# Qervas/cn_chess_ai

Measured on AMD Instinct MI355X. Metric: env steps/sec + DQN updates/sec at 8192 parallel games, 1/2/4/8 MI355X, higher is better.
Workload: dtype f32

## Files before the change

### cn_chess_ai_amd/csrc/xq_refine.hip.h

```cpp
#pragma once

namespace xq {

constexpr float kScreenEps = 0.0078125f * 1.0625f;
constexpr float kScreenBiasEps = 0.001953125f;
enum { kScreenCheckEvery = 32, kScreenHoldSteps = 512 };
constexpr double kScreenMaxPairs = 24.0, kScreenMaxWhole = 1.0;

__device__ __forceinline__ int float_order_key(float f) {
    const int b = __builtin_bit_cast(int, f);
    return b ^ ((b >> 31) & 0x7fffffff);
}
__device__ __forceinline__ float float_from_key(int k) { return __builtin_bit_cast(float, k ^ ((k >> 31) & 0x7fffffff)); }
__device__ __forceinline__ float wave_sum_f32(float v) {
#pragma unroll
    for (int off = 32; off >= 1; off >>= 1) v += __shfl_xor(v, off, 64);
    return v;
}

enum { kRefineSamples = 32, kRefineMaxPerThread = 64 };

template <int KFIX>
__device__ __forceinline__ float quarter_dot(const float* __restrict__ ap, const float* __restrict__ wp, int K, int ql) {
    float acc = 0.f;
    if (KFIX > 0) {
        constexpr int NT = KFIX > 0 ? KFIX / 64 : 1;
        float4 x[NT], w[NT];
#pragma unroll
        for (int t = 0; t < KFIX / 64; ++t) {
            x[t] = *reinterpret_cast<const float4*>(ap + t * 64 + ql * 4);
            w[t] = *reinterpret_cast<const float4*>(wp + t * 64 + ql * 4);
        }
#pragma unroll
        for (int t = 0; t < KFIX / 64; ++t) {
            acc = fmaf(x[t].x, w[t].x, acc); acc = fmaf(x[t].y, w[t].y, acc);
            acc = fmaf(x[t].z, w[t].z, acc); acc = fmaf(x[t].w, w[t].w, acc);
        }
    } else {
        for (int k = ql * 4; k < K; k += 64) {
            const float4 x = *reinterpret_cast<const float4*>(ap + k);
            const float4 w = *reinterpret_cast<const float4*>(wp + k);
            acc = fmaf(x.x, w.x, acc); acc = fmaf(x.y, w.y, acc); acc = fmaf(x.z, w.z, acc); acc = fmaf(x.w, w.w, acc);
        }
    }
    return acc;
}
__device__ __forceinline__ float quarter_sum(float v) {
#pragma unroll
    for (int off = 8; off >= 1; off >>= 1) v += __shfl_xor(v, off, 64);
    return v;
}
__device__ __forceinline__ int screen_row(int g, int code) {
    const int q = code & 15;
    return (g >> 2) * 128 + ((g >> 1) & 1) * 64 + 4 * (g & 1) + (code >> 4) * 32 + (q & 3) + 8 * (q >> 2);
}

template <int KFIX, int NPT>
__global__ __launch_bounds__(256) void qmax_refine_kernel(const float* __restrict__ P1, const float* __restrict__ P2, int G, int n, long long ldp,
                                                          const float* __restrict__ a_last, int K, const float* __restrict__ W,
                                                          const float* __restrict__ bias, int NO, unsigned* __restrict__ wm, int parity,
                                                          float* __restrict__ zmax, unsigned long long* __restrict__ stats) {
    extern __shared__ __attribute__((aligned(16))) uint32_t cand[];
    uint16_t* wlist = reinterpret_cast<uint16_t*>(cand + (size_t)G * kRefineSamples);
    __shared__ float sv[8][32];
    __shared__ float na[32], thr[32];
    __shared__ int best[32];
    __shared__ int cnt, nexp;
    const int tid = (int)threadIdx.x;
    const int sl = tid & 31, phase = tid >> 5;
    const int ql = tid & 15, quarter = tid >> 4;
    const int b0 = (int)blockIdx.x * kRefineSamples;
    const int b = b0 + sl;
    const bool ok = b < n;
    if (tid == 0) { cnt = 0; nexp = 0; if (blockIdx.x == 0) { wm[parity ^ 1] = 0u; wm[2 + (parity ^ 1)] = 0u; } }
    unsigned long long st_pairs = 0, st_whole = 0;
    if (tid == 0) { st_pairs = stats[2 * blockIdx.x]; st_whole = stats[2 * blockIdx.x + 1]; }
    if (tid < 32) best[tid] = (int)0x80000000;
    float v[NPT], v2[NPT];
    const int bc = min(b, n - 1);
#pragma unroll
    for (int u = 0; u < NPT; ++u) {
        const int g = min(phase + 8 * u, G - 1);
        v[u] = P1[(long long)g * ldp + bc];
        v2[u] = P2[(long long)g * ldp + bc];
    }
#pragma unroll
    for (int u = 0; u < NPT; ++u)
        if (!ok || phase + 8 * u >= G) { v[u] = kColmaxPadBias; v2[u] = kColmaxPadBias; }
#pragma unroll
    for (int r = 0; r < 2; ++r) {
        const int i = quarter + 16 * r;
        const float* ap = a_last + (long long)min(b0 + i, n - 1) * K;
        const float ss = quarter_sum(quarter_dot<KFIX>(ap, ap, K, ql));
        if (ql == 0) na[i] = ss;
    }
    float m = kColmaxPadBias;
#pragma unroll
    for (int u = 0; u < NPT; ++u) m = fmaxf(m, v[u]);
    sv[phase][sl] = m;
    __syncthreads();
    if (tid < 32) {
        m = sv[0][sl];
#pragma unroll
        for (int p = 1; p < 8; ++p) m = fmaxf(m, sv[p][sl]);
        const float wmx = fmaxf(__builtin_bit_cast(float, wm[parity]), __builtin_bit_cast(float, wm[4]));
        const float bmx = fmaxf(__builtin_bit_cast(float, wm[2 + parity]), __builtin_bit_cast(float, wm[5]));
        const float B = kScreenEps * sqrtf(na[sl]) * wmx + kScreenBiasEps * bmx;
        float t0 = m - 2.f * B * 1.03125f - 1.52587890625e-05f * (fabsf(m) + 2.f * B);
        if (!(t0 == t0)) t0 = -__builtin_inff();
        thr[sl] = b0 + sl < n ? t0 : __builtin_inff();
    }
    __syncthreads();
    {
        const float t = thr[sl];
#pragma unroll
        for (int u = 0; u < NPT; ++u) {
            const int g = phase + 8 * u;
            if (v[u] >= t) {
                if (v2[u] >= t) wlist[atomicAdd(&nexp, 1)] = (uint16_t)(sl | (g << 5));
                else cand[atomicAdd(&cnt, 1)] = (uint32_t)sl | ((uint32_t)screen_row(g, (int)(__builtin_bit_cast(uint32_t, v[u]) & 31u)) << 5);
            }
        }
    }
    __syncthreads();
    const int singles = cnt, wholes = nexp;
    for (int e0 = 0; e0 < singles; e0 += 64) {
        float z[4];
        int s2[4], row[4];
        bool live[4];
#pragma unroll
        for (int r = 0; r < 4; ++r) {
            const int e = e0 + quarter + 16 * r;
            live[r] = e < singles;
            const uint32_t ent = cand[live[r] ? e : 0];
            s2[r] = (int)(ent & 31u);
            row[r] = min((int)(ent >> 5), NO - 1);
            z[r] = quarter_dot<KFIX>(a_last + (long long)(b0 + s2[r]) * K, W + (long long)row[r] * K, K, ql);
        }
#pragma unroll
        for (int r = 0; r < 4; ++r) {
            z[r] = quarter_sum(z[r]) + bias[row[r]];
            if (live[r] && ql == 0 && z[r] == z[r]) atomicMax(&best[s2[r]], float_order_key(z[r]));
        }
    }
    for (int e = 0; e < wholes; ++e) {
        const int ent = wlist[e];
        const int s2 = ent & 31, g = ent >> 5;
        float zb = kColmaxPadBias;
#pragma unroll
        for (int r = 0; r < 2; ++r) {
            const int row = screen_row(g, quarter + 16 * r);
            const int rc = min(row, NO - 1);
            const float z = quarter_sum(quarter_dot<KFIX>(a_last + (long long)(b0 + s2) * K, W + (long long)rc * K, K, ql)) + bias[rc];
            if (row < NO) zb = fmaxf(zb, z);
        }
        if (ql == 0) atomicMax(&best[s2], float_order_key(zb));
    }
    __syncthreads();
    if (tid < 32 && ok) zmax[b] = float_from_key(best[sl]);
    if (tid == 0) {
        stats[2 * blockIdx.x] = st_pairs + (unsigned long long)(singles + wholes);
        stats[2 * blockIdx.x + 1] = st_whole + (unsigned long long)wholes;
    }
}

struct TdFused {
    SlotSrc src;
    const int32_t* action_to; const float* reward; const uint8_t* done;
    const float* a_s;
    const float* w_out; const float* b_out;
    const float* view; long long view_ld; int view_kmax;
    float gamma;
    float* dtop; float* dsc; int32_t* act; float* qsa; float* yv; float* lossv;
};
__host__ __device__ inline size_t refine_cand_words(int G) { const size_t w = (size_t)G * 32; return w < 8192 ? 8192 : w; }
__host__ __device__ inline size_t refine_wlist_bytes(int G) { return ((size_t)G * 32 * sizeof(uint16_t) + 15) & ~(size_t)15; }
__host__ __device__ inline size_t refine_stage_bytes() { return (size_t)3 * 32 * 256 * sizeof(float); }
template <int KFIX, bool TD = false, class Loss = SquaredLoss>
__global__ __launch_bounds__(256) void qmax_refine2_kernel(const float* __restrict__ R, int ranges, int gpr ,
                                                           const float* __restrict__ P1, const float* __restrict__ P2, int G, int n, long long ldp,
                                                           const float* __restrict__ na_all, const float* __restrict__ a_last, int K,
                                                           const float* __restrict__ W, const float* __restrict__ bias, int NO,
                                                           unsigned* __restrict__ wm, int parity, float* __restrict__ zmax,
                                                           unsigned long long* __restrict__ stats, const TdFused T, int whole_mode, const Loss L) {
    extern __shared__ __attribute__((aligned(16))) uint32_t cand[];
    uint16_t* wlist = reinterpret_cast<uint16_t*>(cand + refine_cand_words(G));
    __shared__ float sv[8][32];
    __shared__ float thr[32];
    __shared__ int best[32];
    __shared__ int cnt, nexp;
    __shared__ unsigned gbits[256];
    __shared__ unsigned long long gpop[4];
    const int tid = (int)threadIdx.x;
    const int sl = tid & 31, phase = tid >> 5;
    const int ql = tid & 15, quarter = tid >> 4;
    const int b0 = (int)blockIdx.x * kRefineSamples;
    const int b = b0 + sl;
    const bool ok = b < n;
    const int bc = min(b, n - 1);
    if (tid == 0) { cnt = 0; nexp = 0; if (blockIdx.x == 0) { wm[parity ^ 1] = 0u; wm[2 + (parity ^ 1)] = 0u; } }
    unsigned long long st_pairs = 0, st_whole = 0;
    if (tid == 0) { st_pairs = stats[2 * blockIdx.x]; st_whole = stats[2 * blockIdx.x + 1]; }
    if (tid < 32) best[tid] = (int)0x80000000;
    const bool stage_ok = KFIX > 0 && G <= 256;
    gbits[tid] = 0u;
    const int td_lane = tid & 63, td_w = tid >> 6;
    int td_a = -1; float td_r = 0.f, td_bo = 0.f; bool td_dn = false;
    float zq[8];
    if (TD) {
        static_assert(!TD || KFIX == 256, "fused TD delta: 256-wide last hidden layer");
        if (td_lane < 8) {
            const int bb = min(b0 + td_w * 8 + td_lane, n - 1);
            const int sslot = slot_of(T.src, bb);
            td_a = T.action_to[sslot];
            td_r = T.reward[sslot];
            td_dn = T.done[sslot] != 0;
            td_bo = T.b_out[(td_a >= 0 && td_a < 96) ? td_a : 0];
        }
#pragma unroll
        for (int i = 0; i < 8; ++i) {
            const int bb = min(b0 + td_w * 8 + i, n - 1);
            const int a = __shfl(td_a, i, 64);
            const int ac = (a >= 0 && a < 96) ? a : 0;
            const float4 av = *reinterpret_cast<const float4*>(T.a_s + (long long)bb * 256 + td_lane * 4);
            const float4 wv = *reinterpret_cast<const float4*>(T.w_out + (long long)ac * 256 + td_lane * 4);
            zq[i] = (av.x * wv.x + av.y * wv.y) + (av.z * wv.z + av.w * wv.w);
        }
    }
    float m = kColmaxPadBias;
    for (int r = phase; r < ranges; r += 8) m = fmaxf(m, R[(long long)r * ldp + bc]);
    sv[phase][sl] = m;
    __syncthreads();
    if (tid < 32) {
        m = sv[0][sl];
#pragma unroll
        for (int p = 1; p < 8; ++p) m = fmaxf(m, sv[p][sl]);
        const float wmx = fmaxf(__builtin_bit_cast(float, wm[parity]), __builtin_bit_cast(float, wm[4]));
        const float bmx = fmaxf(__builtin_bit_cast(float, wm[2 + parity]), __builtin_bit_cast(float, wm[5]));
        const float B = kScreenEps * sqrtf(na_all[bc]) * wmx + kScreenBiasEps * bmx;
        float t0 = m - 2.f * B * 1.03125f - 1.52587890625e-05f * (fabsf(m) + 2.f * B);
        if (!(t0 == t0)) t0 = -__builtin_inff();
        thr[sl] = ok ? t0 : __builtin_inff();
    }
    __syncthreads();
    {
        const float t = thr[sl];
        for (int r = phase; r < ranges; r += 8) {
            if (R[(long long)r * ldp + bc] < t) continue;
            const int g0 = r * gpr, g1 = min(G, g0 + gpr);
            for (int g = g0; g < g1; g += 16) {
                float v[16], v2[16];
#pragma unroll
                for (int u = 0; u < 16; ++u) v[u] = P1[(long long)min(g + u, g1 - 1) * ldp + bc];
#pragma unroll
                for (int u = 0; u < 16; ++u) v2[u] = (g + u < g1 && v[u] >= t) ? P2[(long long)(g + u) * ldp + bc] : 0.f;
#pragma unroll
                for (int u = 0; u < 16; ++u) {
                    if (g + u < g1 && v[u] >= t) {
                        if (v2[u] >= t) { wlist[atomicAdd(&nexp, 1)] = (uint16_t)(sl | ((g + u) << 5)); if (stage_ok) atomicOr(&gbits[g + u], 1u << sl); }
                        else cand[atomicAdd(&cnt, 1)] = (uint32_t)sl | ((uint32_t)screen_row(g + u, (int)(__builtin_bit_cast(uint32_t, v[u]) & 31u)) << 5);
                    }
                }
            }
        }
    }
    __syncthreads();
    const int singles = cnt, wholes = nexp;
    for (int e0 = 0; e0 < singles; e0 += 64) {
        float z[4];
        int s2[4], row[4];
        bool live[4];
#pragma unroll
        for (int r = 0; r < 4; ++r) {
            const int e = e0 + quarter + 16 * r;
            live[r] = e < singles;
            const uint32_t ent = cand[live[r] ? e : 0];
            s2[r] = (int)(ent & 31u);
            row[r] = min((int)(ent >> 5), NO - 1);
            z[r] = quarter_dot<KFIX>(a_last + (long long)(b0 + s2[r]) * K, W + (long long)row[r] * K, K, ql);
        }
#pragma unroll
        for (int r = 0; r < 4; ++r) {
            z[r] = quarter_sum(z[r]) + bias[row[r]];
            if (live[r] && ql == 0 && z[r] == z[r]) atomicMax(&best[s2[r]], float_order_key(z[r]));
        }
    }
    const bool staged_pass = stage_ok && KFIX == 256 && wholes >= 8 && whole_mode == 2;
    if (staged_pass) {
        float* Wt0 = reinterpret_cast<float*>(cand);
        float* At = reinterpret_cast<float*>(reinterpret_cast<unsigned char*>(wlist) + refine_wlist_bytes(G));
        {
            const unsigned long long m = __ballot(__popc(gbits[tid]) >= 8);
            if ((tid & 63) == 0) gpop[tid >> 6] = m;
        }
        __syncthreads();
        unsigned long long gm[4] = {gpop[0], gpop[1], gpop[2], gpop[3]};
        bool a_staged = false;
        for (;;) {
            int gs[3];
#pragma unroll
            for (int u = 0; u < 3; ++u) {
                gs[u] = -1;
#pragma unroll
                for (int wv = 0; wv < 4; ++wv)
                    if (gs[u] < 0 && gm[wv]) { gs[u] = wv * 64 + __builtin_ctzll(gm[wv]); gm[wv] &= gm[wv] - 1; }
            }
            if (gs[0] < 0) break;
            float bj[3][2];
#pragma unroll
            for (int u = 0; u < 3; ++u)
#pragma unroll
                for (int r = 0; r < 2; ++r) bj[u][r] = gs[u] >= 0 ? bias[min(screen_row(gs[u], quarter + 16 * r), NO - 1)] : 0.f;
#pragma unroll
            for (int half = 0; half < 2; ++half) {
                float4 ra[4], rw0[4], rw1[4], rw2[4];
#pragma unroll
                for (int q = 0; q < 4; ++q) {
                    const int i = (half * 4 + q) * 256 + tid, j = i >> 6, c = i & 63;
                    ra[q] = *reinterpret_cast<const float4*>(a_last + (long long)min(b0 + j, n - 1) * K + 4 * c);
                    rw0[q] = *reinterpret_cast<const float4*>(W + (long long)min(screen_row(gs[0], j), NO - 1) * K + 4 * c);
                    rw1[q] = *reinterpret_cast<const float4*>(W + (long long)min(screen_row(gs[1] >= 0 ? gs[1] : gs[0], j), NO - 1) * K + 4 * c);
                    rw2[q] = *reinterpret_cast<const float4*>(W + (long long)min(screen_row(gs[2] >= 0 ? gs[2] : gs[0], j), NO - 1) * K + 4 * c);
                }
#pragma unroll
                for (int q = 0; q < 4; ++q) {
                    const int i = (half * 4 + q) * 256 + tid;
                    if (!a_staged) reinterpret_cast<float4*>(At)[i] = ra[q];
                    if (gs[0] >= 0) reinterpret_cast<float4*>(Wt0)[i] = rw0[q];
                    if (gs[1] >= 0) reinterpret_cast<float4*>(At + 1 * 32 * 256)[i] = rw1[q];
                    if (gs[2] >= 0) reinterpret_cast<float4*>(At + 2 * 32 * 256)[i] = rw2[q];
                }
            }
            a_staged = true;
            __syncthreads();
#pragma unroll
            for (int u = 0; u < 3; ++u) {
                if (gs[u] < 0) continue;
                const float* Wt = u == 0 ? Wt0 : At + u * 32 * 256;
                unsigned left = gbits[gs[u]];
                while (left) {
                    const int s2 = __builtin_ctz(left);
                    left &= left - 1;
                    float zb = kColmaxPadBias;
#pragma unroll
                    for (int r = 0; r < 2; ++r) {
                        const int j = quarter + 16 * r;
                        const float z = quarter_sum(quarter_dot<KFIX>(At + s2 * 256, Wt + j * 256, K, ql)) + bj[u][r];
                        if (screen_row(gs[u], j) < NO) zb = fmaxf(zb, z);
                    }
                    if (ql == 0) atomicMax(&best[s2], float_order_key(zb));
                }
            }
            __syncthreads();
        }
    }
    for (int e = 0; e < wholes; ++e) {
        const int ent = wlist[e];
        const int s2 = ent & 31, g = ent >> 5;
        if (staged_pass && __popc(gbits[g]) >= 8) continue;
        float zb = kColmaxPadBias;
#pragma unroll
        for (int r = 0; r < 2; ++r) {
            const int row = screen_row(g, quarter + 16 * r);
            const int rc = min(row, NO - 1);
            const float z = quarter_sum(quarter_dot<KFIX>(a_last + (long long)(b0 + s2) * K, W + (long long)rc * K, K, ql)) + bias[rc];
            if (row < NO) zb = fmaxf(zb, z);
        }
        if (ql == 0) atomicMax(&best[s2], float_order_key(zb));
    }
    __syncthreads();
    if (tid < 32 && ok) zmax[b] = float_from_key(best[sl]);
    if (tid == 0) {
        stats[2 * blockIdx.x] = st_pairs + (unsigned long long)(singles + wholes);
        stats[2 * blockIdx.x + 1] = st_whole + (unsigned long long)wholes;
    }
    if (TD) {
        float4 av[8], vv[8];
#pragma unroll
        for (int i = 0; i < 8; ++i) {
            const int bb = min(b0 + td_w * 8 + i, n - 1);
            const int a = __shfl(td_a, i, 64);
            const bool has_view = a >= 0 && a < 96 && a < T.view_kmax;
            av[i] = *reinterpret_cast<const float4*>(T.a_s + (long long)bb * 256 + td_lane * 4);
            vv[i] = has_view ? *reinterpret_cast<const float4*>(T.view + (long long)a * T.view_ld + td_lane * 4) : make_float4(0.f, 0.f, 0.f, 0.f);
        }
#pragma unroll
        for (int i = 0; i < 8; ++i) {
            const int bb = b0 + td_w * 8 + i;
            const int a = __shfl(td_a, i, 64);
            const float r = __shfl(td_r, i, 64), bo = __shfl(td_bo, i, 64);
            const bool dn = __shfl((int)td_dn, i, 64) != 0;
            const bool live = a >= 0 && a < 96;
            float z = zq[i];
#pragma unroll
            for (int off = 32; off > 0; off >>= 1) z += __shfl_xor(z, off, 64);
            const float zm = float_from_key(best[td_w * 8 + i]);
            float q = 0.f, y = 0.f, delta = 0.f;
            if (live) {
                q = tanhf(z + bo);
                y = dn ? r : r + T.gamma * tanhf(zm);
                delta = L.err(q - y) * td_dtanh(q) * 1.f;
            }
            if (bb < n) {
                float4 o = make_float4(0.f, 0.f, 0.f, 0.f);
                if (live && a < T.view_kmax) {
                    o.x = delta * vv[i].x * (1.f - av[i].x * av[i].x); o.y = delta * vv[i].y * (1.f - av[i].y * av[i].y);
                    o.z = delta * vv[i].z * (1.f - av[i].z * av[i].z); o.w = delta * vv[i].w * (1.f - av[i].w * av[i].w);
                }
                *reinterpret_cast<float4*>(T.dtop + (long long)bb * 256 + td_lane * 4) = o;
                if (td_lane == 0) {
                    T.dsc[bb] = delta;
                    T.act[bb] = live ? a : -1;
                    T.qsa[bb] = q; T.yv[bb] = y;
                    T.lossv[bb] = live ? L.loss(q - y) : 0.f;
                }
            }
        }
    }
}


}
```

Measured before the change: 47.85 million.

## Restructure refine kernel to hoist loads, drop a barrier, and batch screening reads

Result: faster. 48.75 million, median of 6 (+1.9%).

```diff
diff --git a/cn_chess_ai_amd/csrc/xq_refine.hip.h b/cn_chess_ai_amd/csrc/xq_refine.hip.h
--- a/cn_chess_ai_amd/csrc/xq_refine.hip.h
+++ b/cn_chess_ai_amd/csrc/xq_refine.hip.h
@@ -176,7 +176,43 @@
 __host__ __device__ inline size_t refine_cand_words(int G) { const size_t w = (size_t)G * 32; return w < 8192 ? 8192 : w; }
 __host__ __device__ inline size_t refine_wlist_bytes(int G) { return ((size_t)G * 32 * sizeof(uint16_t) + 15) & ~(size_t)15; }
 __host__ __device__ inline size_t refine_stage_bytes() { return (size_t)3 * 32 * 256 * sizeof(float); }
-template <int KFIX, bool TD = false, class Loss = SquaredLoss>
+#ifdef XQ_REFINE_PROBE
+__device__ unsigned long long* refine_dbg;
+__device__ __forceinline__ unsigned long long refine_clock() {
+    unsigned long long t;
+    asm volatile("s_waitcnt vmcnt(0) lgkmcnt(0)\n\ts_memtime %0\n\ts_waitcnt lgkmcnt(0)" : "=s"(t) :: "memory");
+    return t;
+}
+__device__ __forceinline__ unsigned long long refine_realtime() { return __builtin_amdgcn_s_memrealtime(); }
+__device__ __forceinline__ void refine_stamp_out(int k, unsigned long long v) { refine_dbg[(size_t)blockIdx.x * 16 + k] = v; }
+#else
+__device__ __forceinline__ unsigned long long refine_clock() { return 0ull; }
+__device__ __forceinline__ unsigned long long refine_realtime() { return 0ull; }
+__device__ __forceinline__ void refine_stamp_out(int, unsigned long long) {}
+#endif
+struct RefineChunk { float v[16], w[16]; };
+__device__ __forceinline__ unsigned refine_chunk_last(bool on, int g, int g1) { return on && g1 > g ? (unsigned)(g1 - 1 - g) : 0u; }
+__device__ __forceinline__ void refine_chunk_p1(RefineChunk& c, const float* __restrict__ P1s, bool on, int g, int g1, unsigned ld) {
+    const float* base = P1s + (unsigned long long)(unsigned)(on && g1 > g ? g : 0) * ld;
+    const unsigned last = refine_chunk_last(on, g, g1);
+#pragma unroll
+    for (unsigned u = 0; u < 16; ++u) c.v[u] = base[(unsigned long long)min(u, last) * ld];
+}
+template <bool EAGER>
+__device__ __forceinline__ void refine_chunk_p2(RefineChunk& c, const float* __restrict__ P2s, bool on, int g, int g1, unsigned ld, float t) {
+    const float* base = P2s + (unsigned long long)(unsigned)(on && g1 > g ? g : 0) * ld;
+    const unsigned last = refine_chunk_last(on, g, g1);
+#pragma unroll
+    for (unsigned u = 0; u < 16; ++u) {
+        if (EAGER) c.w[u] = base[(unsigned long long)min(u, last) * ld];
+        else c.w[u] = base[(unsigned long long)((u <= last && c.v[u] >= t) ? u : 0u) * ld];
+    }
+}
+__device__ __forceinline__ void refine_chunk_pin(float (&x)[16]) {
+#pragma unroll
+    for (int u = 0; u < 16; ++u) asm volatile("" : "+v"(x[u]));
+}
+template <int KFIX, bool TD = false, class Loss = SquaredLoss, int DBG = 0>
 __global__ __launch_bounds__(256) void qmax_refine2_kernel(const float* __restrict__ R, int ranges, int gpr ,
                                                            const float* __restrict__ P1, const float* __restrict__ P2, int G, int n, long long ldp,
                                                            const float* __restrict__ na_all, const float* __restrict__ a_last, int K,
@@ -186,18 +222,28 @@
     extern __shared__ __attribute__((aligned(16))) uint32_t cand[];
     uint16_t* wlist = reinterpret_cast<uint16_t*>(cand + refine_cand_words(G));
     __shared__ float sv[8][32];
-    __shared__ float thr[32];
     __shared__ int best[32];
     __shared__ int cnt, nexp;
     __shared__ unsigned gbits[256];
     __shared__ unsigned long long gpop[4];
     const int tid = (int)threadIdx.x;
+    unsigned long long stp[13] = {0, 0, 0, 0, 0, 0, 0, 0, 0, 0, 0, 0, 0};
+    if (DBG & 1) { stp[11] = refine_realtime(); stp[0] = refine_clock(); }
     const int sl = tid & 31, phase = tid >> 5;
     const int ql = tid & 15, quarter = tid >> 4;
     const int b0 = (int)blockIdx.x * kRefineSamples;
     const int b = b0 + sl;
     const bool ok = b < n;
     const int bc = min(b, n - 1);
+    const bool two = ranges <= 16 && gpr <= 16;
+    float r0 = kColmaxPadBias, r1 = kColmaxPadBias;
+    float m = kColmaxPadBias;
+    if (two) {
+        r0 = R[(long long)min(phase, ranges - 1) * ldp + bc];
+        r1 = R[(long long)min(phase + 8, ranges - 1) * ldp + bc];
+    }
+    const float na_b = na_all[bc];
+    const unsigned wm_w = wm[parity], wm_ws = wm[4], wm_b = wm[2 + parity], wm_bs = wm[5];
     if (tid == 0) { cnt = 0; nexp = 0; if (blockIdx.x == 0) { wm[parity ^ 1] = 0u; wm[2 + (parity ^ 1)] = 0u; } }
     unsigned long long st_pairs = 0, st_whole = 0;
     if (tid == 0) { st_pairs = stats[2 * blockIdx.x]; st_whole = stats[2 * blockIdx.x + 1]; }
@@ -205,8 +251,7 @@
     const bool stage_ok = KFIX > 0 && G <= 256;
     gbits[tid] = 0u;
     const int td_lane = tid & 63, td_w = tid >> 6;
-    int td_a = -1; float td_r = 0.f, td_bo = 0.f; bool td_dn = false;
-    float zq[8];
+    int td_a = -1; float td_r = 0.f, td_bo = 0.f; unsigned td_dn = 0u;
     if (TD) {
         static_assert(!TD || KFIX == 256, "fused TD delta: 256-wide last hidden layer");
         if (td_lane < 8) {
@@ -214,60 +259,118 @@
             const int sslot = slot_of(T.src, bb);
             td_a = T.action_to[sslot];
             td_r = T.reward[sslot];
-            td_dn = T.done[sslot] != 0;
-            td_bo = T.b_out[(td_a >= 0 && td_a < 96) ? td_a : 0];
-        }
+            td_dn = T.done[sslot];
+        }
+    }
+    if (two) {
+        if (phase < ranges) m = fmaxf(m, r0);
+        if (phase + 8 < ranges) m = fmaxf(m, r1);
+    } else {
+        for (int r = phase; r < ranges; r += 8) m = fmaxf(m, R[(long long)r * ldp + bc]);
+    }
+    sv[phase][sl] = m;
+    if (DBG & 1) stp[1] = refine_clock();
+    __syncthreads();
+    if (DBG & 1) stp[2] = refine_clock();
+    float4 tav[8], twv[8], tvv[8];
+    if (TD) {
+        if (td_lane < 8) td_bo = T.b_out[(td_a >= 0 && td_a < 96) ? td_a : 0];
 #pragma unroll
         for (int i = 0; i < 8; ++i) {
             const int bb = min(b0 + td_w * 8 + i, n - 1);
             const int a = __shfl(td_a, i, 64);
             const int ac = (a >= 0 && a < 96) ? a : 0;
-            const float4 av = *reinterpret_cast<const float4*>(T.a_s + (long long)bb * 256 + td_lane * 4);
-            const float4 wv = *reinterpret_cast<const float4*>(T.w_out + (long long)ac * 256 + td_lane * 4);
-            zq[i] = (av.x * wv.x + av.y * wv.y) + (av.z * wv.z + av.w * wv.w);
-        }
-    }
-    float m = kColmaxPadBias;
-    for (int r = phase; r < ranges; r += 8) m = fmaxf(m, R[(long long)r * ldp + bc]);
-    sv[phase][sl] = m;
-    __syncthreads();
-    if (tid < 32) {
+            const float* vp = (a >= 0 && a < 96 && a < T.view_kmax) ? T.view + (long long)a * T.view_ld : T.w_out;
+            tav[i] = *reinterpret_cast<const float4*>(T.a_s + (long long)bb * 256 + td_lane * 4);
+            twv[i] = *reinterpret_cast<const float4*>(T.w_out + (long long)ac * 256 + td_lane * 4);
+            tvv[i] = *reinterpret_cast<const float4*>(vp + td_lane * 4);
+        }
+    }
+    if (DBG & 1) stp[3] = refine_clock();
+    float t;
+    {
         m = sv[0][sl];
 #pragma unroll
         for (int p = 1; p < 8; ++p) m = fmaxf(m, sv[p][sl]);
-        const float wmx = fmaxf(__builtin_bit_cast(float, wm[parity]), __builtin_bit_cast(float, wm[4]));
-        const float bmx = fmaxf(__builtin_bit_cast(float, wm[2 + parity]), __builtin_bit_cast(float, wm[5]));
-        const float B = kScreenEps * sqrtf(na_all[bc]) * wmx + kScreenBiasEps * bmx;
+        const float wmx = fmaxf(__builtin_bit_cast(float, wm_w), __builtin_bit_cast(float, wm_ws));
+        const float bmx = fmaxf(__builtin_bit_cast(float, wm_b), __builtin_bit_cast(float, wm_bs));
+        const float B = kScreenEps * sqrtf(na_b) * wmx + kScreenBiasEps * bmx;
         float t0 = m - 2.f * B * 1.03125f - 1.52587890625e-05f * (fabsf(m) + 2.f * B);
         if (!(t0 == t0)) t0 = -__builtin_inff();
-        thr[sl] = ok ? t0 : __builtin_inff();
-    }
-    __syncthreads();
+        t = ok ? t0 : __builtin_inff();
+    }
     {
-        const float t = thr[sl];
-        for (int r = phase; r < ranges; r += 8) {
-            if (R[(long long)r * ldp + bc] < t) continue;
-            const int g0 = r * gpr, g1 = min(G, g0 + gpr);
-            for (int g = g0; g < g1; g += 16) {
-                float v[16], v2[16];
-#pragma unroll
-                for (int u = 0; u < 16; ++u) v[u] = P1[(long long)min(g + u, g1 - 1) * ldp + bc];
-#pragma unroll
-                for (int u = 0; u < 16; ++u) v2[u] = (g + u < g1 && v[u] >= t) ? P2[(long long)(g + u) * ldp + bc] : 0.f;
-#pragma unroll
-                for (int u = 0; u < 16; ++u) {
-                    if (g + u < g1 && v[u] >= t) {
-                        if (v2[u] >= t) { wlist[atomicAdd(&nexp, 1)] = (uint16_t)(sl | ((g + u) << 5)); if (stage_ok) atomicOr(&gbits[g + u], 1u << sl); }
-                        else cand[atomicAdd(&cnt, 1)] = (uint32_t)sl | ((uint32_t)screen_row(g + u, (int)(__builtin_bit_cast(uint32_t, v[u]) & 31u)) << 5);
-                    }
-                }
-            }
-        }
-    }
-    __syncthreads();
+        const float *P1s = P1 + bc, *P2s = P2 + bc;
+        const unsigned ld = (unsigned)ldp;
+        const auto emit = [&](const RefineChunk& c, bool on, int g, int g1) {
+#pragma unroll
+            for (int u = 0; u < 16; ++u) {
+                if (on && g + u < g1 && c.v[u] >= t) {
+                    if (c.w[u] >= t) { wlist[atomicAdd(&nexp, 1)] = (uint16_t)(sl | ((g + u) << 5)); if (stage_ok) atomicOr(&gbits[g + u], 1u << sl); }
+                    else cand[atomicAdd(&cnt, 1)] = (uint32_t)sl | ((uint32_t)screen_row(g + u, (int)(__builtin_bit_cast(uint32_t, c.v[u]) & 31u)) << 5);
+                }
+            }
+        };
+        constexpr bool EAGER = (DBG & 2) != 0;
+        if (two) {
+            const bool hit0 = phase < ranges && !(r0 < t), hit1 = phase + 8 < ranges && !(r1 < t);
+            const int ga = phase * gpr, gb = (phase + 8) * gpr;
+            const int ea = hit0 ? min(G, ga + gpr) : ga, eb = hit1 ? min(G, gb + gpr) : gb;
+            if (hit0 || hit1) {
+                RefineChunk ca, cb;
+                refine_chunk_p1(ca, P1s, hit0, ga, ea, ld);
+                refine_chunk_p1(cb, P1s, hit1, gb, eb, ld);
+                if (EAGER) { refine_chunk_p2<true>(ca, P2s, hit0, ga, ea, ld, t); refine_chunk_p2<true>(cb, P2s, hit1, gb, eb, ld, t); }
+                __builtin_amdgcn_sched_barrier(0);
+                if (DBG & 1) stp[4] = refine_clock();
+                refine_chunk_pin(ca.v); refine_chunk_pin(cb.v);
+                if (!EAGER) {
+                    refine_chunk_p2<false>(ca, P2s, hit0, ga, ea, ld, t); refine_chunk_p2<false>(cb, P2s, hit1, gb, eb, ld, t);
+                    __builtin_amdgcn_sched_barrier(0);
+                }
+                if (DBG & 1) stp[5] = refine_clock();
+                refine_chunk_pin(ca.w); refine_chunk_pin(cb.w);
+                emit(ca, hit0, ga, ea);
+                emit(cb, hit1, gb, eb);
+            }
+        } else {
+            for (int r = phase; r < ranges; r += 8) {
+                if (R[(long long)r * ldp + bc] < t) continue;
+                const int g0 = r * gpr, g1 = min(G, g0 + gpr);
+                for (int g = g0; g < g1; g += 16) {
+                    RefineChunk c;
+                    refine_chunk_p1(c, P1s, true, g, g1, ld);
+                    refine_chunk_pin(c.v);
+                    refine_chunk_p2<EAGER>(c, P2s, true, g, g1, ld, t);
+                    refine_chunk_pin(c.w);
+                    emit(c, true, g, g1);
+                }
+            }
+#if defined(__HIP_DEVICE_COMPILE__) && !defined(__gfx950__)
+#error "qmax_refine2_kernel: the s_waitcnt immediate below is encoded for gfx950"
+#endif
+            __builtin_amdgcn_s_waitcnt(0x0F70);
+        }
+    }
+    if (DBG & 1) { stp[6] = refine_clock(); if (stp[4] == 0) stp[4] = stp[5] = stp[6]; }
+    float td_q = 0.f;
+    if (TD) {
+        float zmine = 0.f;
+#pragma unroll
+        for (int i = 0; i < 8; ++i) {
+            const float4 av = tav[i], wv = twv[i];
+            float z = (av.x * wv.x + av.y * wv.y) + (av.z * wv.z + av.w * wv.w);
+#pragma unroll
+            for (int off = 32; off > 0; off >>= 1) z += __shfl_xor(z, off, 64);
+            if (td_lane == i) zmine = z;
+        }
+        if (td_lane < 8 && td_a >= 0 && td_a < 96) td_q = tanhf(zmine + td_bo);
+    }
+    __syncthreads();
+    if (DBG & 1) stp[7] = refine_clock();
     const int singles = cnt, wholes = nexp;
     for (int e0 = 0; e0 < singles; e0 += 64) {
-        float z[4];
+        float z[4], bj[4];
         int s2[4], row[4];
         bool live[4];
 #pragma unroll
@@ -277,14 +380,16 @@
             const uint32_t ent = cand[live[r] ? e : 0];
             s2[r] = (int)(ent & 31u);
             row[r] = min((int)(ent >> 5), NO - 1);
+            bj[r] = bias[row[r]];
             z[r] = quarter_dot<KFIX>(a_last + (long long)(b0 + s2[r]) * K, W + (long long)row[r] * K, K, ql);
         }
 #pragma unroll
         for (int r = 0; r < 4; ++r) {
-            z[r] = quarter_sum(z[r]) + bias[row[r]];
+            z[r] = quarter_sum(z[r]) + bj[r];
             if (live[r] && ql == 0 && z[r] == z[r]) atomicMax(&best[s2[r]], float_order_key(z[r]));
         }
     }
+    if (DBG & 1) stp[8] = refine_clock();
     const bool staged_pass = stage_ok && KFIX == 256 && wholes >= 8 && whole_mode == 2;
     if (staged_pass) {
         float* Wt0 = reinterpret_cast<float*>(cand);
@@ -359,65 +464,67 @@
         const int s2 = ent & 31, g = ent >> 5;
         if (staged_pass && __popc(gbits[g]) >= 8) continue;
         float zb = kColmaxPadBias;
+        float bj[2];
+#pragma unroll
+        for (int r = 0; r < 2; ++r) bj[r] = bias[min(screen_row(g, quarter + 16 * r), NO - 1)];
 #pragma unroll
         for (int r = 0; r < 2; ++r) {
             const int row = screen_row(g, quarter + 16 * r);
             const int rc = min(row, NO - 1);
-            const float z = quarter_sum(quarter_dot<KFIX>(a_last + (long long)(b0 + s2) * K, W + (long long)rc * K, K, ql)) + bias[rc];
+            const float z = quarter_sum(quarter_dot<KFIX>(a_last + (long long)(b0 + s2) * K, W + (long long)rc * K, K, ql)) + bj[r];
             if (row < NO) zb = fmaxf(zb, z);
         }
         if (ql == 0) atomicMax(&best[s2], float_order_key(zb));
     }
     __syncthreads();
+    if (DBG & 1) stp[9] = refine_clock();
     if (tid < 32 && ok) zmax[b] = float_from_key(best[sl]);
     if (tid == 0) {
         stats[2 * blockIdx.x] = st_pairs + (unsigned long long)(singles + wholes);
         stats[2 * blockIdx.x + 1] = st_whole + (unsigned long long)wholes;
     }
     if (TD) {
-        float4 av[8], vv[8];
-#pragma unroll
-        for (int i = 0; i < 8; ++i) {
-            const int bb = min(b0 + td_w * 8 + i, n - 1);
-            const int a = __shfl(td_a, i, 64);
-            const bool has_view = a >= 0 && a < 96 && a < T.view_kmax;
-            av[i] = *reinterpret_cast<const float4*>(T.a_s + (long long)bb * 256 + td_lane * 4);
-            vv[i] = has_view ? *reinterpret_cast<const float4*>(T.view + (long long)a * T.view_ld + td_lane * 4) : make_float4(0.f, 0.f, 0.f, 0.f);
+        const bool mine = td_a >= 0 && td_a < 96;
+        float q = 0.f, y = 0.f, delta = 0.f;
+        if (td_lane < 8) {
+            const float zm = float_from_key(best[td_w * 8 + td_lane]);
+            const float r = td_r;
+            const bool dn = td_dn != 0u;
+            if (mine) {
+                q = td_q;
+                y = dn ? r : r + T.gamma * tanhf(zm);
+                delta = L.err(q - y) * td_dtanh(q) * 1.f;
+            }
+            const int bb = b0 + td_w * 8 + td_lane;
+            if (bb < n) {
+                T.dsc[bb] = delta;
+                T.act[bb] = mine ? td_a : -1;
+                T.qsa[bb] = q; T.yv[bb] = y;
+                T.lossv[bb] = mine ? L.loss(q - y) : 0.f;
+            }
         }
 #pragma unroll
         for (int i = 0; i < 8; ++i) {
             const int bb = b0 + td_w * 8 + i;
             const int a = __shfl(td_a, i, 64);
-            const float r = __shfl(td_r, i, 64), bo = __shfl(td_bo, i, 64);
-            const bool dn = __shfl((int)td_dn, i, 64) != 0;
+            const float dl = __shfl(delta, i, 64);
             const bool live = a >= 0 && a < 96;
-            float z = zq[i];
-#pragma unroll
-            for (int off = 32; off > 0; off >>= 1) z += __shfl_xor(z, off, 64);
-            const float zm = float_from_key(best[td_w * 8 + i]);
-            float q = 0.f, y = 0.f, delta = 0.f;
-            if (live) {
-                q = tanhf(z + bo);
-                y = dn ? r : r + T.gamma * tanhf(zm);
-                delta = L.err(q - y) * td_dtanh(q) * 1.f;
-            }
             if (bb < n) {
                 float4 o = make_float4(0.f, 0.f, 0.f, 0.f);
                 if (live && a < T.view_kmax) {
-                    o.x = delta * vv[i].x * (1.f - av[i].x * av[i].x); o.y = delta * vv[i].y * (1.f - av[i].y * av[i].y);
-                    o.z = delta * vv[i].z * (1.f - av[i].z * av[i].z); o.w = delta * vv[i].w * (1.f - av[i].w * av[i].w);
+                    o.x = dl * tvv[i].x * (1.f - tav[i].x * tav[i].x); o.y = dl * tvv[i].y * (1.f - tav[i].y * tav[i].y);
+                    o.z = dl * tvv[i].z * (1.f - tav[i].z * tav[i].z); o.w = dl * tvv[i].w * (1.f - tav[i].w * tav[i].w);
                 }
                 *reinterpret_cast<float4*>(T.dtop + (long long)bb * 256 + td_lane * 4) = o;
-                if (td_lane == 0) {
-                    T.dsc[bb] = delta;
-                    T.act[bb] = live ? a : -1;
-                    T.qsa[bb] = q; T.yv[bb] = y;
-                    T.lossv[bb] = live ? L.loss(q - y) : 0.f;
-                }
-            }
-        }
-    }
-}
-
-
-}
+            }
+        }
+    }
+    if (DBG & 1) {
+        stp[10] = refine_clock(); stp[12] = refine_realtime();
+        if (tid == 0)
+#pragma unroll
+            for (int k = 0; k < 13; ++k) refine_stamp_out(k, stp[k]);
+    }
+}
+
+}
```
